# 54rt1n/shardmerge

Hardware: AMD Instinct MI355X
Metric: merged-weight GB/s per GPU + % HBM roofline, Llama-3-70B 3-way FFT merge (higher is better)
Workload: dtype f32; 1 GPU; Llama-3-70B block tensors, this rank's 1/8 slice (9 per block x 10 blocks), K=3 finetunes, bf16 in/out, resident in HBM; workload_id=llama3-70b-slice, k=3, parallelism=tensor-partition x1 (no data-path collective), streams_per_gpu=8

## Files before the change

shardmerge_amd/csrc/sm_capi.inc:

```

struct smhip_ctx {
    smhip::Pipeline<SM_BACKEND> pipe;
    explicit smhip_ctx(int device) : pipe(device) {}
};

#define SM_GUARD(ctx)                      \
    if (!(ctx)) return SMHIP_ERR_ARG;      \
    (ctx)->pipe.err.clear();
#define SM_FINISH(ctx, rc)                                                        \
    do {                                                                          \
        int rc__ = (rc);                                                          \
        if (rc__ == SMHIP_OK && !(ctx)->pipe.be.ok()) {                           \
            (ctx)->pipe.err = (ctx)->pipe.be.error();                             \
            rc__ = SMHIP_ERR_HIP;                                                 \
        }                                                                         \
        return rc__;                                                              \
    } while (0)

template <class Desc, class Scalars>
static int delta_tensor_check(smhip_ctx* ctx, const char* op, const Desc* d, const void* out, const float* delta_out,
                              bool need_base, Scalars scalars) {
    auto bad = [&](const char* what) { return ctx->pipe.fail(SMHIP_ERR_ARG, std::string(op) + ": " + what); };
    if (!d) return bad("null descriptor");
    if (d->k < 1 || d->k > SMHIP_MAX_MODELS) return bad("k out of range (1..16)");
// ... 350 lines not shown
                             void* stream) {
    SM_GUARD(ctx);
    if (!x || !norm_out) return ctx->pipe.fail(SMHIP_ERR_ARG, "bad argument");
    if (dtype < SMHIP_BF16 || dtype > SMHIP_F32) return ctx->pipe.fail(SMHIP_ERR_ARG, "bad dtype");
    ctx->pipe.stream = stream;
    const int rc0 = ctx->pipe.reserve(1, 1);
    if (rc0) SM_FINISH(ctx, rc0);
    smhip::SigDesc sg{x, base, dtype, 1.f};
    double out = 0;
    if (!ctx->pipe.run_serial_norms(&sg, 1, n, &out))
        return ctx->pipe.fail(SMHIP_ERR_ARG, "reference_cpu norm: inputs must be 16-byte aligned");
    *norm_out = (float)out;
    SM_FINISH(ctx, SMHIP_OK);
}

int smhip_debug_option(smhip_ctx* ctx, const char* key, long value) {
    SM_GUARD(ctx);
    if (key && std::string(key) == "aten_overlap") { ctx->pipe.aten_overlap = value != 0; return SMHIP_OK; }
    if (key && std::string(key) == "emf_max_sample") { ctx->pipe.emf_max_sample = value >= 1 && value <= 4096 ? (int)value : smhip::EMF_MAX_SAMPLE; return SMHIP_OK; }
    if (key && std::string(key) == "aten_serial") { ctx->pipe.aten_serial = value != 0; return SMHIP_OK; }
    if (key && std::string(key) == "class_norms") { ctx->pipe.class_norms_mode = value >= 0 && value <= 2 ? (int)value : 1; return SMHIP_OK; }
    if (key && std::string(key) == "cand_cap") { ctx->pipe.debug_cand_cap = value > 0 ? (uint32_t)value : 0u; return SMHIP_OK; }
    if (key && std::string(key) == "sel_chunks") { ctx->pipe.debug_sel_chunks = value > 0 ? (uint32_t)value : 0u; return SMHIP_OK; }
    if (key && std::string(key) == "sel_flush_always") { ctx->pipe.debug_flush_always = value != 0; return SMHIP_OK; }
    if (key && std::string(key) == "fuse_norms") { ctx->pipe.fuse_norms = value != 0; return SMHIP_OK; }
    if (key && std::string(key) == "noise_seed") { ctx->pipe.noise_seed_base = (uint32_t)value; return SMHIP_OK; }
    if (key && std::string(key) == "spectral_intermediates") { ctx->pipe.spectral_inter = value != 0; return SMHIP_OK; }
    if (key && std::string(key) == "fuse_spec_norm") { ctx->pipe.fuse_spec_norm = value != 0; return SMHIP_OK; }
    if (key && std::string(key) == "sel_wgs_per_cu") { ctx->pipe.sel_wgs_per_cu = value > 0 ? (int)value : 5; return SMHIP_OK; }
    if (key && std::string(key) == "pair1d") { ctx->pipe.pair1d_enabled = value != 0; return SMHIP_OK; }
    if (key && std::string(key) == "spec_cull") { ctx->pipe.spec_cull = value != 0; return SMHIP_OK; }
    if (key && std::string(key) == "spec_min_bins") { ctx->pipe.spec_min_bins = value >= 0 ? (size_t)value : (size_t)1 << 20; return SMHIP_OK; }
    if (key && std::string(key) == "dftp_pairs") { ctx->pipe.dftp_pairs_enabled = value != 0; return SMHIP_OK; }
    if (key && std::string(key) == "f2s_pair") { ctx->pipe.f2s_pair = value != 0; return SMHIP_OK; }
    if (key && std::string(key) == "f1_multi") { ctx->pipe.f1_multi = value != 0; return SMHIP_OK; }
    if (key && std::string(key) == "force_bluestein") { ctx->pipe.debug_force_bluestein = value != 0; return SMHIP_OK; }
    if (key && std::string(key) == "force_split") { ctx->pipe.debug_force_split = value > 1 && value <= smhip::DFTP_MAX_P ? (int)value : 0; return SMHIP_OK; }
    if (key && std::string(key) == "fold_columns") { ctx->pipe.fold_enabled = value != 0; return SMHIP_OK; }
    if (key && std::string(key) == "della_slab_rows") { ctx->pipe.della_slab_rows = value > 0 ? (size_t)value : 0; return SMHIP_OK; }
    if (key && std::string(key) == "fold_min_rows") { ctx->pipe.fold_min_rows = value > 0 ? (int)value : SM_FOLD_MIN_ROWS; return SMHIP_OK; }
    return ctx->pipe.fail(SMHIP_ERR_ARG, "unknown debug option");
}

int smhip_debug_query(smhip_ctx* ctx, const char* key, long* value) {
    SM_GUARD(ctx);
    if (!key || !value) return SMHIP_ERR_ARG;
    if (std::string(key) == "spec_hit") { *value = ctx->pipe.last_spec_verdict(); SM_FINISH(ctx, SMHIP_OK); }
    if (std::string(key) == "spec_checked" || std::string(key) == "spec_hits") {
        unsigned long long c = 0, h = 0;
        ctx->pipe.spec_totals(&c, &h);
        *value = (long)(std::string(key) == "spec_hits" ? h : c);
        SM_FINISH(ctx, SMHIP_OK);
    }
    if (std::string(key) == "aten_fast" || std::string(key) == "aten_group" || std::string(key) == "aten_slow") {
        unsigned long long v3[3];
        ctx->pipe.aten_stats(1, v3);
        *value = (long)v3[std::string(key) == "aten_fast" ? 0 : std::string(key) == "aten_group" ? 1 : 2];
        SM_FINISH(ctx, SMHIP_OK);
    }
    return ctx->pipe.fail(SMHIP_ERR_ARG, "unknown debug query");
}

int smhip_profile_enable(smhip_ctx* ctx, int on) { SM_GUARD(ctx); ctx->pipe.be.profile_enable(on != 0); return SMHIP_OK; }
int smhip_profile_reset(smhip_ctx* ctx) { SM_GUARD(ctx); ctx->pipe.be.profile_reset(); return SMHIP_OK; }
int smhip_profile_count(smhip_ctx* ctx) { return ctx ? ctx->pipe.be.profile_count() : 0; }
int smhip_profile_get(smhip_ctx* ctx, int i, const char** name, uint64_t* launches, double* total_ms) {
    SM_GUARD(ctx);
    return ctx->pipe.be.profile_get(i, name, launches, total_ms) ? SMHIP_OK : SMHIP_ERR_ARG;
}

}
```

shardmerge_amd/csrc/sm_kernels.hpp:

```cpp
#pragma once
#include <cmath>
#include <cstring>

#include "fft_engine.hpp"
#include "sm_aten_core.hpp"

namespace smhip {

struct cf4 { float x, y, z, w; };
struct u32x4 { uint32_t x, y, z, w; };

enum { DT_BF16 = 0, DT_F16 = 1, DT_F32 = 2 };

struct SigDesc {
    const void* x;
    const void* base;
    int dtype;
    float prescale;
};

SM_HD uint32_t umax(uint32_t a, uint32_t b) { return a > b ? a : b; }
SM_HD float u2f(uint32_t u) { float f; memcpy(&f, &u, 4); return f; }
SM_HD uint32_t f2u(float f) { uint32_t u; memcpy(&u, &f, 4); return u; }
SM_HD float bf16_to_f(uint32_t h) { return u2f(h << 16); }
// ... 882 lines not shown
    }
}

#ifndef SM_COL_THREADS
#define SM_COL_THREADS 512
#endif
constexpr int f2_bins_for(int T, int N = 1 << 30) {
    if (T == 64 && N <= 256) return 8;
    return (SM_COL_THREADS / (2 * T)) > 1 ? (SM_COL_THREADS / (2 * T) > 8 ? 8 : SM_COL_THREADS / (2 * T)) : 1;
}
#ifndef SM_I1_THREADS
constexpr int i1_bins_for(int T) { return 2; }
#else
constexpr int i1_bins_for(int T) { return (SM_I1_THREADS / T) > 2 ? ((SM_I1_THREADS / T) > 16 ? 16 : (SM_I1_THREADS / T)) : 2; }
#endif
template <class P> constexpr int f2_bins() { if constexpr (P::is_static) return f2_bins_for(P::T, P::N); else return 1; }
template <class P> constexpr int i1_bins() { if constexpr (P::is_static) return i1_bins_for(P::T); else return 2; }

struct F2SParams {
    FftPlanDev plan;
    const cf4* t1;
    int pitch4;
    int R, C, Cb;
    int role_a;
    float scale;
    float* re; float* im;
    unsigned long long* hist;
    int slab, Cb_real, Rfull;
    size_t slab_elems;
    double* im_partials;
    SliceGrid sl;
    int two;
    const cf4* t1_2; int role_a_2; float scale_2; float* re_2;
};
template <class P> constexpr int f2s_groups() {
    if constexpr (P::is_static) return f2_nsig_for(P::T) == 2 ? 2 * f2_bins_for(P::T, P::N) : 1; else return 1;
}

#ifndef SM_F2S_ILV
#define SM_F2S_ILV 1
#endif
constexpr int F2S_ILV = SM_F2S_ILV;
#ifndef SM_F2S_DIRECT
#define SM_F2S_DIRECT 0
#endif
template <class P, int G> constexpr int f2s_direct() {
    if constexpr (!P::is_static) return 0;
    else {
        constexpr int R0 = P::radix(0);
        constexpr bool ok = F2S_ILV == 1 && (G == 1 || G == 2) && P::npass >= 2 && P::T % 2 == 0 && R0 % 2 == 0 &&
                            (P::N / R0) % 2 == 0 && (EMAX / R0) * R0 * P::T >= P::N;
        return ok ? (SM_F2S_DIRECT & 3) : 0;
    }
}
template <class P, int G, bool FOLD = false, class Ex>
SM_HD void k_f2s(Ex& ex, const F2SParams& p) {
    if constexpr (FOLD && !fold_col_plan<P>()) { return; } else {
    typename Ex::template State<FftState> st;
    ex.init(st);
    float* lds = ex.lds() + LDS_SCRATCH_FLOATS;
    const FftPlanDev& pl = p.plan;
    const int T = plan_T<P>(pl), R = plan_N<P>(pl);
    const int LF = plan_lds<P>(pl);
    constexpr int XG = G >= 8 ? 1 : 8 / G;
    int bid_in_slice;
    const int slice = slice_of(ex, p.sl, bid_in_slice);
    int sig2 = 0;
    const int lbid = p.two ? pick_signal(2, bid_in_slice, XG, sig2) : xcd_remap(bid_in_slice, XG);
    const cf4* const t1 = (sig2 ? p.t1_2 : p.t1) + slice * p.sl.t1_stride;
    const size_t pl_off = slice * p.sl.plane_stride;
    const int role_a_ = sig2 ? p.role_a_2 : p.role_a;
    const float scale_ = sig2 ? p.scale_2 : p.scale;
    float* const re_ = sig2 ? p.re_2 : p.re;
    const int kbase = lbid * G;
    if (kbase >= p.Cb) {
        if (p.im_partials) ex.each(st, [&](int tid, FftState&) { if (tid == 0) p.im_partials[ex.bid()] = 0.0; });
        return;
    }
    const int nthreads = G * T;
    const int half = R / 2;
    uint32_t* lhist = (uint32_t*)(lds + G * LF);

    constexpr int DIRECT = f2s_direct<P, G>();
    if constexpr ((DIRECT & 1) != 0) {
        constexpr int R0 = P::radix(0), MB0 = EMAX / R0, nb0 = P::N / R0;
        ex.each(st, [&](int tid, FftState& s) {
            const int g = tid / T, t = tid % T;
            const int k2 = kbase + g;
            const int kc = k2 < p.Cb ? k2 : p.Cb - 1;
            const int par = t & 1;
            static_for<0, MB0>([&](auto m_c) {
                constexpr int m = decltype(m_c)::value;
                const bool live = (t + m * T) < nb0 && k2 < p.Cb;
                static_for<0, R0 / 2>([&](auto q_c) {
                    constexpr int q = decltype(q_c)::value;
                    const int pm = live ? (t >> 1) + m * (T / 2) + q * nb0 + par * (nb0 / 2) : 0;
                    cf4 v;
#if defined(SM_DIAG_NOMEM)
                    v = cf4{(float)q, (float)t, 1.f, (float)kc};
#else
                    if constexpr (FOLD) v = t1[(size_t)(kc / p.slab) * p.slab_elems + (size_t)pm * p.slab + (kc % p.slab)];
                    else v = t1[(size_t)pm * p.pitch4 + kc];
#endif
                    s.xr[m * R0 + 2 * q] = live ? v.x : 0.f; s.xi[m * R0 + 2 * q] = live ? v.y : 0.f;
                    s.xr[m * R0 + 2 * q + 1] = live ? v.z : 0.f; s.xi[m * R0 + 2 * q + 1] = live ? v.w : 0.f;
                });
// ... 55 lines not shown
#pragma unroll
                for (int c = 0; c < 4; ++c) {
                    const int k1 = 4 * (t + u * T) + c;
                    if (k1 < R) o[4 * u + c] = l[lpad(k1)];
                }
            }
        });

    ex.each(st, [&](int tid, FftState& s) {
        const int g = tid / T, t = tid % T;
        const int k2 = kbase + g;
        s.red[0] = 0.0;
        if (k2 >= p.Cb) return;
        const float sc = scale_;
        size_t poff = (size_t)k2 * R;
        int kreal = k2;
        if constexpr (FOLD) { kreal = fold_bin(k2, p.slab, p.Cb_real, R, p.Rfull, poff); if (kreal < 0) return; }
        const uint32_t w = (uint32_t)bin_weight(kreal, p.C);
        float* dre = re_ + pl_off + poff;
        float* dim = p.im + pl_off + poff;
        float imsq = 0.f;
        if constexpr ((DIRECT & 2) != 0) {
            constexpr int RL = P::radix(P::npass - 1), MBL = EMAX / RL, NsL = P::N / RL;
            static_for<0, MBL>([&](auto m_c) {
                constexpr int m = decltype(m_c)::value;
                const int j = t + m * T;
                if (j < NsL) {
                    static_for<0, RL>([&](auto i_c) {
                        constexpr int i = decltype(i_c)::value, e = m * RL + i;
                        const float vr = s.xr[e] * sc;
#if defined(SM_DIAG_NOMEM)
                        if (vr == 12345.678f)
#endif
                        dre[j + i * NsL] = vr;
                        if (role_a_) {
                            const float vi = s.xi[e] * sc;
#if defined(SM_DIAG_NOMEM)
                            if (vi == 12345.678f)
#endif
                            dim[j + i * NsL] = vi;
                            imsq += vi * vi;
                        }
                        if (p.hist) ex.lds_atomic_add(&lhist[(f2u(vr) & 0x7fffffffu) >> 20], w);
                    });
                }
            });
        } else
#pragma unroll
        for (int u = 0; u < EMAX / 4; ++u) {
            const int k0 = 4 * (t + u * T);
            if (k0 + 3 < R && (R & 3) == 0) {
                cf4 vr = {s.xr[4 * u] * sc, s.xr[4 * u + 1] * sc, s.xr[4 * u + 2] * sc, s.xr[4 * u + 3] * sc};
#if defined(SM_DIAG_NOMEM)
                if (vr.x == 12345.678f)
#endif
                *(cf4*)(dre + k0) = vr;
                if (role_a_) {
                    cf4 vi = {s.xi[4 * u] * sc, s.xi[4 * u + 1] * sc, s.xi[4 * u + 2] * sc, s.xi[4 * u + 3] * sc};
#if defined(SM_DIAG_NOMEM)
                    if (vi.x == 12345.678f)
#endif
                    *(cf4*)(dim + k0) = vi;
                    imsq += vi.x * vi.x + vi.y * vi.y + vi.z * vi.z + vi.w * vi.w;
                }
            } else {
#pragma unroll
                for (int c = 0; c < 4; ++c) {
                    if (k0 + c < R) {
                        dre[k0 + c] = s.xr[4 * u + c] * sc;
                        if (role_a_) { const float vi = s.xi[4 * u + c] * sc; dim[k0 + c] = vi; imsq += vi * vi; }
                    }
                }
            }
            if (p.hist) {
#pragma unroll
                for (int c = 0; c < 4; ++c) {
                    if (k0 + c < R) {
                        const uint32_t key = f2u(s.xr[4 * u + c] * sc) & 0x7fffffffu;
                        ex.lds_atomic_add(&lhist[key >> 20], w);
                    }
                }
            }
        }
        s.red[0] = (double)imsq * (double)w;
    });
    if (p.hist) {
        ex.sync();
        ex.each(st, [&](int tid, FftState&) {
            for (int h = tid; h < HIST1_BINS; h += nthreads) {
                const uint32_t v = lhist[h];
                if (v) ex.global_atomic_add(&p.hist[h], (unsigned long long)v);
            }
        });
    }
    if (p.im_partials) {
        ex.sync();
        ex.template block_sum<1>(st, [&](const double* tot) { p.im_partials[ex.bid()] = tot[0]; });
    }
    }
}

template <class Ex>
SM_HD void k_f2_r1(Ex& ex, const F2Params& p) {
// ... 1435 lines not shown
            sr += qr; si += qi2;
        }
        s.red[0] = sr; s.red[1] = si;
    });
    ex.template block_sum<2>(st, [&](const double* tot) {
        p.partials[2 * (size_t)ex.bid()] = tot[0];
        p.partials[2 * (size_t)ex.bid() + 1] = tot[1];
    });
}

SM_HD uint32_t hash_u32(uint32_t x) {
    x ^= x >> 16; x *= 0x7feb352du; x ^= x >> 15; x *= 0x846ca68bu; x ^= x >> 16;
    return x;
}
SM_HD float model_noise(uint32_t seed, size_t i, float sigma) {
    const uint32_t h1 = hash_u32((uint32_t)i * 2u + 1u + seed * 0x9e3779b9u) ^ hash_u32((uint32_t)(i >> 31) + seed);
    const uint32_t h2 = hash_u32(h1 + 0x68bc21ebu);
    if ((h2 >> 24) < 21u) return 0.f;
    const float s4 = (float)(h1 & 0xffffu) + (float)(h1 >> 16) + (float)(h2 & 0xffffu) + (float)(hash_u32(h2) >> 16);
    return sigma * 1.7320508f * (s4 * (1.0f / 65536.0f) - 2.0f);
}

struct SpecRescaleParams {
    const float* re; const float* im;
    float* dre; float* dim;
    int R, C, Cb;
    int vec4;
    float thr;
    float scale;
    float sigma; uint32_t seed;
    unsigned long long* hist;
    int chunks;
    double* im_partials;
};
template <class Ex>
SM_HD void k_spec_rescale(Ex& ex, const SpecRescaleParams& p) {
    typename Ex::template State<EmptyState> st;
    ex.init(st);
    uint32_t* lh = (uint32_t*)(ex.lds() + LDS_SCRATCH_FLOATS);
    const int nt = ex.nthreads();
    const size_t total = (size_t)p.Cb * p.R;
    const size_t nquad = (total + 3) / 4;
    const WeightRanges wr = weight_ranges(p.R, p.C, p.Cb);
    if (p.hist) {
        ex.each(st, [&](int tid, EmptyState&) { for (int b = tid; b < HIST1_BINS; b += nt) lh[b] = 0; });
        ex.sync();
    }
    ex.each(st, [&](int tid, EmptyState& s) {
        double imacc = 0.0;
        const size_t start = (size_t)ex.bid() * p.chunks * nt;
        for (int c = 0; c < p.chunks; ++c) {
            const size_t qi = start + (size_t)c * nt + tid;
            if (qi >= nquad) break;
            const size_t i0 = 4 * qi;
            float a[4], b[4] = {0.f, 0.f, 0.f, 0.f};
            const int n = load_quad(p.re, i0, total, p.vec4, a);
            if (p.im) load_quad(p.im, i0, total, p.vec4, b);
            float r[4], im[4];
#pragma unroll
            for (int e = 0; e < 4; ++e) {
                r[e] = (fabsf(a[e]) < p.thr) ? model_noise(p.seed, i0 + e, p.sigma) : a[e] * p.scale;
                im[e] = b[e] * p.scale;
            }
            if (p.vec4) {
                cf4 v = {r[0], r[1], r[2], r[3]};
                *(cf4*)(p.dre + i0) = v;
                if (p.im) { cf4 vi = {im[0], im[1], im[2], im[3]}; *(cf4*)(p.dim + i0) = vi; }
            } else {
                for (int e = 0; e < n; ++e) { p.dre[i0 + e] = r[e]; if (p.im) p.dim[i0 + e] = im[e]; }
            }
            if (p.hist) {
#pragma unroll
                for (int e = 0; e < 4; ++e)
                    if (e < n) ex.lds_atomic_add(&lh[(f2u(r[e]) & 0x7fffffffu) >> 20], weight_at(wr, i0 + e));
            }
            if (p.im_partials) {
                float q = 0.f;
#pragma unroll
                for (int e = 0; e < 4; ++e)
                    if (e < n) q += (float)weight_at(wr, i0 + e) * im[e] * im[e];
                imacc += q;
            }
        }
        s.red[0] = imacc;
    });
    if (p.hist) {
        ex.sync();
        ex.each(st, [&](int tid, EmptyState&) {
            for (int b = tid; b < HIST1_BINS; b += nt) {
                const uint32_t v = lh[b];
                if (v) ex.global_atomic_add(&p.hist[b], (unsigned long long)v);
            }
        });
    }
    if (p.im_partials) {
        ex.sync();
        ex.template block_sum<1>(st, [&](const double* tot) { p.im_partials[ex.bid()] = tot[0]; });
    }
}

constexpr int NORMS_MAX = 16;
constexpr int NORMS_K = 8;
// ... 1210 lines not shown
```

shardmerge_amd/csrc/sm_pipeline.hpp:

```cpp
#pragma once
#include <algorithm>
#include <cmath>
#include <cstdio>
#include <map>
#include <string>
#include <vector>

#include "../../include/shardmerge_hip.h"
#include "sm_kernels.hpp"
#include "sm_aten_norm.hpp"
#include "sm_bluestein.hpp"
#include "sm_lora.hpp"
#include "sm_ties.hpp"
#include "sm_dare.hpp"
#include "sm_breadcrumbs.hpp"
#include "sm_geo.hpp"
#include "sm_sce.hpp"
#include "sm_della.hpp"
#include "sm_consensus.hpp"

namespace smhip {

#define SM_KERNEL_TAG(Tag, ParamsT, NAME, CALL)                                      \
    struct Tag {                                                                     \
// ... 292 lines not shown
};

struct ProfEntry { std::string name; uint64_t launches = 0; double ms = 0; };

inline size_t round_up(size_t v, size_t m) { return (v + m - 1) / m * m; }

struct PairOut {
    void* out = nullptr; int out_mode = OUT_F32;
    const void* base = nullptr; int base_dtype = DT_BF16;
    float post = 1.f;
    int ifft_policy = 1;
};

template <class B>
class Pipeline {
  public:
    B be;
    std::string err;
    void* stream = nullptr;
    uint32_t debug_cand_cap = 0;
    uint32_t debug_sel_chunks = 0;
    bool debug_flush_always = false;
    bool spec_cull = true;
    size_t spec_min_bins = 1 << 20;
    bool dftp_pairs_enabled = true;
    int debug_force_split = 0;
    int sel_wgs_per_cu = 5;
    bool safe_select = false;
    uint32_t noise_seed_base = 0;
    bool spectral_inter = true;
    bool f2s_pair = true;
    size_t f2s_pair_max_bins = (size_t)64 << 20;
    bool f1_multi = true;
    bool fuse_spec_norm = true;
    float noise_sigma = 1.2e-7f;

    explicit Pipeline(int device) : be(device) {}
    ~Pipeline() {
        for (auto& kv : plans_) if (kv.second.dev.tw) be.free((void*)kv.second.dev.tw);
        for (Buffer* b : {&cand_, &t1_, &small_, &tmpA_, &tmpB_, &tmpC_, &fullS_, &saveR_, &saveI_, &aten_, &emf_, &lora_, &dora_, &ties_}) if (b->p) be.free(b->p);
        for (Buffer& b : pool_) if (b.p) be.free(b.p);
        if (mail_) be.free_host(mail_);
        for (Buffer& b : inter_) if (b.p) be.free(b.p);
        for (Buffer& b : rowspec_) if (b.p) be.free(b.p);
        for (Buffer& b : tr_) if (b.p) be.free(b.p);
        for (auto& kv : rough_tw_) if (kv.second) be.free(kv.second);
        for (auto& kv : blue_) { if (kv.second.chirp) be.free(kv.second.chirp); if (kv.second.filt) be.free(kv.second.filt); }
    }

    int fail(int code, const std::string& msg) { err = msg; return code; }

    int get_plan(int N, FftPlanDev& out) {
        auto it = plans_.find(N);
        if (it == plans_.end()) {
            HostPlan hp;
            int T;
            std::vector<int> rad;
            if (plan_shape(N, T, rad)) {
                hp.ok = true;
                hp.dev.N = N; hp.dev.T = T; hp.dev.npass = (int)rad.size();
                for (int i = 0; i < MAX_PASSES; ++i) hp.dev.radix[i] = i < (int)rad.size() ? rad[i] : 1;
                hp.dev.cx = plan_uses_cx(N) ? 1 : 0;
                hp.dev.lds_floats = hp.dev.cx ? (int)round_up((size_t)2 * (N + (N >> 4) + 1), 32)
                                              : (int)round_up((size_t)lpad(N) + 1, 32);
                std::vector<cf2> tw(N);
                for (int j = 0; j < N; ++j) {
// ... 383 lines not shown
            return SMHIP_OK;
        }
        const int xgs = p.ilv > p.nb ? p.ilv / p.nb : 1;
        const bool joint = joint_rows(g);
        const int nlaunch = joint ? 1 : g.batch;
        if (joint) p.R = g.R * g.rough / 2;
        const int grid = (int)round_up((size_t)(p.R + p.nb - 1) / p.nb, 8 * xgs);
        if (multi && (nlaunch != 1 || g.rough > 1 || (size_t)grid * 2 * nm > PART_DOUBLES || !p.vec)) return SMHIP_ERR_ARG;
        if ((size_t)grid * 2 * nlaunch > PART_DOUBLES) return fail(SMHIP_ERR_SHAPE, "too many rows");
        const size_t lds = (LDS_SCRATCH_FLOATS + (size_t)p.nb * p.plan.lds_floats) * 4;
        cf4* const t1base = p.t1;
        double* const pbase = p.partials;
        if (multi) {
            for (int i = 0; i < nm; ++i) multi->partials[i] = pbase + (size_t)i * 2 * grid;
            multi->b_off = (long long)((size_t)g.C * dt_size(sig.dtype));
            p.sigs = *multi;
            launch_fft<KF1>(p.plan, grid * nm, p.nb * p.plan.T, lds, p, true);
            if (grid_out) *grid_out = grid;
            return SMHIP_OK;
        }
        for (int bi = 0; bi < nlaunch; ++bi) {
            p.a = sig_at(a, (size_t)bi * g.R * g.C); p.b = sig_at(b, (size_t)bi * g.R * g.C);
            p.t1 = t1base + (size_t)bi * (g.t1_slice / 2);
            p.partials = pbase + (size_t)bi * 2 * grid;
            if (blue) { F1BParams q; q.f = p; q.bt = bt; launch_fft<KF1B>(p.plan, grid, p.plan.T, lds, q); }
            else launch_fft<KF1>(p.plan, grid, p.nb * p.plan.T, lds, p, p.vec != 0);
        }
        if (grid_out) *grid_out = grid * nlaunch;
        if (g.rough > 1) return run_dftp(g, t1base, true, F2S_ILV, g.pitch4, g.t1_slice / 2, false);
        return SMHIP_OK;
    }
    struct F2SSecond { const void* t1; bool role_a; float scale; };
    int run_f2s(const Geo& g, bool role_a, float scale, bool hist, const void* t1buf = nullptr, int* im_parts = nullptr,
                const F2SSecond* second = nullptr) {
        F2SParams p;
        p.two = 0; p.t1_2 = nullptr; p.role_a_2 = 0; p.scale_2 = 0.f; p.re_2 = nullptr;
        if (second) {
            if (g.batch != 1 || second->role_a == role_a) return fail(SMHIP_ERR_ARG, "internal: paired column pass");
            p.two = 1; p.t1_2 = (const cf4*)second->t1; p.role_a_2 = second->role_a ? 1 : 0; p.scale_2 = second->scale;
            p.re_2 = plane(g, second->role_a ? P_REA : P_REB);
        }
        const int nsg = second ? 2 : 1;
        const int Rt = g.R / g.fold;
        int rc = get_plan(Rt, p.plan);
        if (rc) return rc;
        p.t1 = (const cf4*)(t1buf ? t1buf : t1_.p); p.pitch4 = g.pitch4 * g.fold; p.R = Rt; p.C = g.C;
        p.Cb = g.fold == 4 ? 4 * g.pitch4 : g.C / 2 + 1;
        p.slab = g.pitch4; p.Cb_real = g.C / 2 + 1; p.Rfull = g.R; p.slab_elems = fold_slab_elems(g, true);
        p.role_a = role_a ? 1 : 0; p.scale = scale;
        p.re = plane(g, role_a ? P_REA : P_REB); p.im = plane(g, P_IMA);
        p.hist = hist ? d_hist() : nullptr;
        const bool st = is_static_plan(p.plan);
        const int G = st ? (f2_nsig_for(p.plan.T) == 2 ? 2 * f2_bins_for(p.plan.T, p.plan.N) : 1) : 1;
        const int xg = G >= 8 ? 1 : 8 / G;
        const int grid = (int)round_up((size_t)(p.Cb + G - 1) / G, 8 * xg) * nsg;
        const size_t lds = (LDS_SCRATCH_FLOATS + (size_t)G * p.plan.lds_floats + HIST1_BINS) * 4;
        const bool any_a = role_a || (second && second->role_a);
        const bool want_im = im_parts && any_a && (size_t)grid * g.batch <= PART_IM_DOUBLES;
        if (im_parts) *im_parts = want_im ? grid * g.batch : -1;
        p.im_partials = want_im ? d_part_im() : nullptr;
        if (g.fold == 4) { launch_fft<KF2SQ>(p.plan, grid, G * p.plan.T, lds, p); return SMHIP_OK; }
        if (g.batch > 1) { p.sl.wgs = grid; p.sl.t1_stride = g.t1_slice / 2; p.sl.plane_stride = (size_t)(g.C / 2 + 1) * g.R; }
        launch_fft<KF2S>(p.plan, grid * g.batch, G * p.plan.T, lds, p);
        return SMHIP_OK;
    }
    void run_spec_norm(const Geo& g, const float* re, const float* im, const float* thr, double& sre, double& sim) {
        const size_t total = (size_t)g.Cb * g.R;
        SpecNormParams q;
        q.re = re; q.im = im; q.R = g.R; q.C = g.Cw; q.Cb = g.Cb; q.vec4 = vec4(g); q.thr = thr;
        q.chunks = pick_chunks((total + 3) / 4, 256, 8, 8);
        int grid = stream_grid((total + 3) / 4, 256, q.chunks);
        while ((size_t)grid * 2 > PART_DOUBLES) { q.chunks *= 2; grid = stream_grid((total + 3) / 4, 256, q.chunks); }
        q.partials = d_part();
        be.template launch<KSpecNorm>(grid, 256, LDS_SCRATCH_FLOATS * 4, q, stream);
        SumPartialsParams sp;
        sp.partials = d_part(); sp.nparts = grid; sp.out = mail_->norm2;
        be.template launch<KSumPartials>(1, 1024, LDS_SCRATCH_FLOATS * 4, sp, stream);
        PublishParams pp;
        pp.flags = d_flags(); pp.thr = d_thr(0); pp.consts = d_consts(); pp.mail = mail_; pp.zero_flags = nullptr;
        be.template launch<KPublish>(1, 64, LDS_SCRATCH_FLOATS * 4, pp, stream);
        be.sync(stream);
        sre = mail_->norm2[0]; sim = mail_->norm2[1];
    }
    void run_spec_rescale(const Geo& g, const float* re, const float* im, float thr, float scale, bool role_a, bool hist,
                          int* im_parts = nullptr) {
        const size_t total = (size_t)g.Cb * g.R;
        SpecRescaleParams q;
        q.re = re; q.im = role_a ? im : nullptr;
        q.dre = plane(g, role_a ? P_REA : P_REB); q.dim = plane(g, P_IMA);
        q.R = g.R; q.C = g.Cw; q.Cb = g.Cb; q.vec4 = vec4(g);
        q.thr = thr; q.scale = scale; q.sigma = noise_sigma; q.seed = ++noise_seed_;
        q.hist = hist ? d_hist() : nullptr;
        q.chunks = pick_chunks((total + 3) / 4, 256, 8, 8);
        const int grid = stream_grid((total + 3) / 4, 256, q.chunks);
        const bool want_im = im_parts && role_a && (size_t)grid <= PART_IM_DOUBLES;
        if (im_parts) *im_parts = want_im ? grid : -1;
        q.im_partials = want_im ? d_part_im() : nullptr;
        be.template launch<KSpecRescale>(grid, 256, (LDS_SCRATCH_FLOATS + HIST1_BINS) * 4, q, stream);
    }
    void run_spec_norm_fused(int sel_parts, int im_parts, double& sre, double& sim) {
        SumsqCandParams sc;
        sc.cand = cand_lists(); sc.thr = d_thr(1); sc.partials = d_part() + 4 * (size_t)sel_parts;
        be.template launch<KSumsqCand>(CAND_GRID, 256, LDS_SCRATCH_FLOATS * 4, sc, stream);
        SumSpecParams sp;
        sp.part4 = d_part(); sp.n4 = sel_parts + CAND_GRID; sp.part1 = d_part_im(); sp.n1 = im_parts; sp.out = mail_->norm2;
        sp.zero_u32 = d_candctr(); sp.zero_u32_count = 3;
        be.template launch<KSumSpec>(1, 1024, LDS_SCRATCH_FLOATS * 4, sp, stream);
        PublishParams pp;
        pp.flags = d_flags(); pp.thr = d_thr(0); pp.consts = d_consts(); pp.mail = mail_; pp.zero_flags = nullptr;
        be.template launch<KPublish>(1, 64, LDS_SCRATCH_FLOATS * 4, pp, stream);
        be.sync(stream);
        sre = mail_->norm2[0]; sim = mail_->norm2[1];
    }

    void read_norms(int grid, double& na, double& nb) {
        SumPartialsParams sp;
        sp.partials = d_part(); sp.nparts = grid; sp.out = mail_->norm2;
        be.template launch<KSumPartials>(1, 1024, LDS_SCRATCH_FLOATS * 4, sp, stream);
        be.sync(stream);
        na = std::sqrt(mail_->norm2[0]); nb = std::sqrt(mail_->norm2[1]);
    }

    int run_f2(const Geo& g, float scale0, float scale1, int swap, bool hist) {
        F2Params p;
        int rc = get_plan(g.R, p.plan);
        if (rc) return rc;
        if (g.R == 1) {
            p.slab = g.pitch4; p.Cb_real = g.C / 2 + 1; p.Rfull = 1; p.slab_elems = 0;
            p.t1 = (const cf4*)t1_.p; p.pitch4 = g.pitch4; p.ilv = 1; p.R = 1; p.C = g.C; p.Cb = g.C / 2 + 1; p.nsig = 2;
            p.swap = swap; p.scale[0] = scale0; p.scale[1] = scale1;
// ... 496 lines not shown
        std::vector<char> used(m, 0);
        std::vector<float> corr((size_t)m * m, 0.f);
        for (int i = 0; i < m; ++i)
            for (int j = i + 1; j < m; ++j) corr[(size_t)i * m + j] = norms[i] * norms[j];
        for (;;) {
            float best = INFINITY;
            bool any = false;
            for (int i = 0; i < m; ++i)
                for (int j = i + 1; j < m; ++j)
                    if (!used[i] && !used[j]) { any = true; best = std::min(best, std::fabs(corr[(size_t)i * m + j])); }
            if (!any) break;
            int bx = -1, by = -1;
            for (int i = 0; i < m && bx < 0; ++i)
                for (int j = i + 1; j < m; ++j)
                    if (!used[i] && !used[j] && std::fabs(corr[(size_t)i * m + j]) == best) { bx = i; by = j; break; }
            if (bx < 0) break;
            out.emplace_back(bx, by);
            used[bx] = used[by] = 1;
        }
        for (int i = 0; i < m; ++i)
            if (!used[i]) out.emplace_back(i, -1);
    }

    struct Slot {
        SigDesc sig;
        double weight;
        double norm;
        bool spectral = false;
        int re_id = -1, im_id = -1;
        float thr = 0.f;
        double spec_scale = 1.0;
        double post = 1.0;
        int rows_id = -1;
    };
    int materialise(const Geo& g, Slot& s, std::vector<char>& inter_busy) {
        if (!s.spectral) return SMHIP_OK;
        const size_t n = (size_t)g.R * g.C;
        int id = -1;
        for (size_t q = 0; q < inter_.size(); ++q) if (!inter_busy[q]) { id = (int)q; break; }
        if (id < 0) { inter_.emplace_back(); inter_busy.push_back(0); id = (int)inter_.size() - 1; }
        int rc = ensure(inter_[id], n * sizeof(float));
        if (rc) return rc;
        inter_busy[id] = 1;
        PairOut po;
        po.out = inter_[id].p; po.out_mode = OUT_F32; po.post = (float)s.post;
        if ((rc = run_inverse(g, (const float*)pool_[s.re_id].p, (const float*)pool_[s.im_id].p, nullptr, po, nullptr, s.thr))) return rc;
        pool_release(s.re_id); pool_release(s.im_id);
        s.spectral = false; s.re_id = s.im_id = -1;
        s.sig = SigDesc{inter_[id].p, nullptr, DT_F32, 1.f};
        return SMHIP_OK;
    }

    bool run_delta_norms(const smhip_layer_desc& d, size_t n, std::vector<Slot>& stack) {
        if (d.k > NORMS_K || d.in_dtype == DT_F32 || (n % 8) != 0) return false;
        DeltaNormsParams p;
        p.k = d.k; p.dtype = d.in_dtype; p.n = n;
        p.ubase[0] = p.ubase[1] = nullptr;
        int nb = 0;
        for (int i = 0; i < NORMS_K; ++i) { p.ft[i] = d.finetune[i < d.k ? i : 0]; p.base_of[i] = 0; }
        for (int i = 0; i < d.k; ++i) {
            if (!d.base[i] || !aligned16(d.base[i]) || !aligned16(d.finetune[i])) return false;
            int j = 0;
            while (j < nb && p.ubase[j] != d.base[i]) ++j;
            if (j == nb) { if (nb == 2) return false; p.ubase[nb++] = d.base[i]; }
            p.base_of[i] = j;
        }
        p.chunks = pick_chunks(n / 8, 256, 4, 8);
        int grid = stream_grid(n / 8, 256, p.chunks);
        while ((size_t)grid * NORMS_MAX > PART_DOUBLES) { p.chunks *= 2; grid = stream_grid(n / 8, 256, p.chunks); }
        p.partials = d_part();
        be.template launch<KDeltaNorms>(grid, 256, LDS_SCRATCH_FLOATS * 4, p, stream);
        SumNParams sp;
        sp.partials = d_part(); sp.nparts = grid; sp.out = mail_->norm2;
        be.template launch<KSumPartialsN>(1, 256, LDS_SCRATCH_FLOATS * 4, sp, stream);
        be.sync(stream);
// ... 410 lines not shown
                return fail(SMHIP_ERR_NONFINITE, buf);
            }
        }
        {
            float acc = 0.f;
            for (int i = 0; i < d.k; ++i) acc += norms32[i];
            mean = (double)(acc / (float)d.k);
        }
        const double target_norm = mean + d.target_norm_offset;
        rp.target_norm = target_norm;
        double cull_pct = d.cull_start_pct;

        std::vector<char> inter_busy(inter_.size(), 0);
        for (size_t q = 0; q < pool_.size(); ++q) {
            bool working = false;
            for (int i = 0; i < 4; ++i) working = working || pidx_[i] == (int)q;
            pool_busy_[q] = working ? 1 : 0;
        }
        noise_seed_ = noise_seed_base;
        int step = 0;
        int round_idx = 0;
        int pair_idx = 0;
        int deferred_step = -1;
        bool deferred_cut = false, deferred_cull = false;
        while (stack.size() > 1) {
            const int m = (int)stack.size();
            std::vector<std::pair<int, int>> pairs;
            correlated_pairs_least(norms32, m, pairs);
            std::vector<Slot> next;
            const bool last_round = (pairs.size() == 1 && pairs[0].second >= 0);
            bool any_pair = false;
            for (auto& pr : pairs) any_pair = any_pair || pr.second >= 0;
            if (!any_pair) { check_flags(false, false); return fail(SMHIP_ERR_NONFINITE, "no pair can be formed (non-finite norms)"); }
            for (auto& pr : pairs) {
                const int x = pr.first, y = pr.second;
                if (step < SMHIP_MAX_PAIRS) { rp.step_x[step] = x; rp.step_y[step] = y; }
                if (y < 0) {
                    next.push_back(stack[x]);
                    if (step < SMHIP_MAX_PAIRS) rp.step_branch[step] = SMHIP_BRANCH_CARRY;
                    ++step;
                    continue;
                }
                Slot A = stack[x], Bs = stack[y];
                const double a_w = stack[x].weight, b_w = stack[y].weight;
                if (A.norm < 0 || Bs.norm < 0) return fail(SMHIP_ERR_ARG, "internal: norm unknown");
                double na = (double)(float)A.norm, nb = (double)(float)Bs.norm;
                bool swapped = false;
                if (std::fabs(na) < std::fabs(nb)) { std::swap(A, Bs); std::swap(na, nb); swapped = true; }
                const double ca = std::fabs(na / target_norm), cb = std::fabs(nb / target_norm);
                const double ratio = cb / (ca + 1e-10);
                PairOut po;
                float* inter = nullptr;
                const bool linear = (nb / (na + 1e-10)) < d.b;
                const bool slerp_proper = !(ca < 1e-6) && !(cb < 1e-6 || ratio < 0.1) && !(nb < 1e-4 || na < 1e-4) && !linear;
                if (last_round) {
                    po = fin;
                } else if (slerp_proper && spectral_ok) {
                } else {
                    int id = -1;
                    for (size_t q = 0; q < inter_.size(); ++q) if (!inter_busy[q]) { id = (int)q; break; }
                    if (id < 0) { inter_.emplace_back(); inter_busy.push_back(0); id = (int)inter_.size() - 1; }
                    Buffer* bb = &inter_[id];
                    if ((rc = ensure(*bb, n * sizeof(float)))) return rc;
                    inter_busy[id] = 1;
                    inter = (float*)bb->p;
                    po.out = inter; po.out_mode = OUT_F32; po.post = 1.f;
// ... 25 lines not shown
                    pa.ifft_policy = 0;
                    if ((rc = pair_arith(A.sig, Bs.sig, R, C, (float)s, (float)(w * s), 1.0, 1, pa, na, nb, &g))) return rc;
                    if (dtmp) {
                        SigDesc ds{dtmp, nullptr, DT_F32, 1.f}, none{nullptr, nullptr, DT_F32, 1.f};
                        run_combine(ds, none, 1.f, 0.f, n, nullptr, &fin, false);
                    }
                    f1_ready = false;
                } else {
                    branch = SMHIP_BRANCH_SLERP;
                    const double t = a_w / (a_w + b_w);
                    if (nb < 1e-4 || na < 1e-4) {
                        SigDesc none{nullptr, nullptr, DT_F32, 1.f};
                        const float sc = (float)(target_norm / na);
                        if (last_round) run_combine(A.sig, none, sc, 0.f, n, delta_out, &po, false);
                        else run_combine(A.sig, none, sc, 0.f, n, inter, nullptr, false);
                        branch = SMHIP_BRANCH_EARLY_V0;
                    } else if (linear) {
                        branch = SMHIP_BRANCH_LINEAR;
                        int grid;
                        if ((rc = run_f1(g, A.sig, Bs.sig, grid))) return rc;
                        f1_ready = false;
                        if ((rc = run_f2_linear(g, (float)(1.0 / na), (float)(1.0 / nb), (float)t))) return rc;
                        PairOut ps = po;
                        ps.post = (float)target_norm;
                        float* dtmp = nullptr;
                        if (last_round && delta_out) { ps = PairOut(); ps.out = delta_out; ps.post = (float)target_norm; dtmp = delta_out; }
                        if ((rc = run_inverse(g, plane(g, P_RER), plane(g, P_IMA), nullptr, ps, last_round ? nullptr : &inv_grid))) return rc;
                        if (dtmp) {
                            SigDesc ds{dtmp, nullptr, DT_F32, 1.f}, none{nullptr, nullptr, DT_F32, 1.f};
                            run_combine(ds, none, 1.f, 0.f, n, nullptr, &fin, false);
                        }
                    } else {
                        int im_parts = -1;
                        const bool any_spec = stack[x].spectral || stack[y].spectral ||
                                              (stack[x].rows_id >= 0 && stack[y].rows_id >= 0);
                        const bool fused1d = !any_spec && pair1d_ok(g);
                        if (fused1d) {
                            f1_ready = false;
                        } else if (!any_spec) {
                            if (!(f1_ready && d.k == 2)) {
                                int grid;
                                if ((rc = run_f1(g, stack[x].sig, stack[y].sig, grid))) return rc;
                            }
                            f1_ready = false;
                            const float s0 = (float)(1.0 / (double)(float)stack[x].norm);
                            const float s1 = (float)(1.0 / (double)(float)stack[y].norm);
                            if ((rc = run_f2(g, s0, s1, swapped ? 1 : 0, d.cutoff_pct > 0))) return rc;
                        } else {
                            f1_ready = false;
                            int* imp = (!last_round && spectral_ok && fuse_spec_norm) ? &im_parts : nullptr;
                            if (f2s_pair && g.batch == 1 && g.fold == 1 && (size_t)g.Cb * g.R <= f2s_pair_max_bins &&
                                !stack[x].spectral && !stack[y].spectral &&
                                stack[x].rows_id >= 0 && stack[y].rows_id >= 0) {
                                const bool xa = !swapped;
                                F2SSecond sec{rowspec_[stack[y].rows_id].p, !xa, (float)(1.0 / (double)(float)stack[y].norm)};
                                if ((rc = run_f2s(g, xa, (float)(1.0 / (double)(float)stack[x].norm), d.cutoff_pct > 0,
                                                  rowspec_[stack[x].rows_id].p, imp, &sec))) return rc;
                            } else
                            for (int side = 0; side < 2; ++side) {
                                const Slot& in = side == 0 ? stack[x] : stack[y];
                                const bool role_a = (side == 0) != swapped;
                                int* ip = role_a ? imp : nullptr;
                                if (in.spectral) {
                                    run_spec_rescale(g, (const float*)pool_[in.re_id].p, (const float*)pool_[in.im_id].p, in.thr,
                                                     (float)in.spec_scale, role_a, d.cutoff_pct > 0, ip);
                                } else if (in.rows_id >= 0) {
                                    if ((rc = run_f2s(g, role_a, (float)(1.0 / (double)(float)in.norm), d.cutoff_pct > 0,
                                                      rowspec_[in.rows_id].p, ip))) return rc;
                                } else {
                                    if ((rc = run_f1_rowpairs(g, in.sig))) return rc;
                                    if ((rc = run_f2s(g, role_a, (float)(1.0 / (double)(float)in.norm), d.cutoff_pct > 0, nullptr, ip))) return rc;
                                }
                            }
                        }
                        bool have_cull;
                        int sel_parts = 0;
                        const bool fused_norm = im_parts > 0 && !safe_select && cull_pct > 0;
                        if (fused1d) have_cull = cull_pct > 0;
                        else spectral_blend(g, BLEND_SLERP, t, d.t_sum, d.cutoff_pct, cull_pct, 1, true, have_cull,
                                            fused_norm ? &sel_parts : nullptr, std::min(pair_idx++, 6));
                        for (int side = 0; side < 2; ++side) {
                            Slot& in = side == 0 ? stack[x] : stack[y];
                            if (in.spectral) { pool_release(in.re_id); pool_release(in.im_id); in.re_id = in.im_id = -1; }
                        }
                        if (!last_round && spectral_ok) {
                            double sre, sim;
                            if (fused_norm && sel_parts > 0) run_spec_norm_fused(sel_parts, im_parts, sre, sim);
                            else run_spec_norm(g, plane(g, P_RER), plane(g, P_IMA), have_cull ? d_thr(1) : nullptr, sre, sim);
                            read_blend_info(&info, d.cutoff_pct > 0, have_cull, true, true);
                            const double ssum = (sre + sim) / ((double)R * (double)C);
                            out_spectral = true;
                            spec_slot = Slot();
                            spec_slot.spectral = true;
                            spec_slot.re_id = pidx_[P_RER]; spec_slot.im_id = pidx_[P_IMA];
                            spec_slot.thr = have_cull ? mail_->thr[1] : 0.f;
                            const double nrm_exact = target_norm * std::sqrt(ssum);
                            const double bias = ref_norms ? aten_gauss_norm_ratio((double)n, nrm_exact / std::sqrt((double)n)) : 1.0;
                            spec_slot.spec_scale = ssum > 0 ? 1.0 / (std::sqrt(ssum) * bias) : 1.0;
                            spec_slot.post = target_norm;
                            spec_slot.norm = nrm_exact * bias;
                            spec_slot.sig = SigDesc{nullptr, nullptr, DT_F32, 1.f};
                            const int r1 = pool_acquire(g.plane_floats * sizeof(float));
                            const int r2 = pool_acquire(g.plane_floats * sizeof(float));
                            if (r1 < 0 || r2 < 0) return SMHIP_ERR_NOMEM;
                            pidx_[P_RER] = r1; pidx_[P_IMA] = r2;
                        } else {
                        PairOut ps = po;
                        ps.post = (float)target_norm;
                        float* dtmp = nullptr;
                        if (last_round && delta_out) { ps = PairOut(); ps.out = delta_out; ps.post = (float)target_norm; dtmp = delta_out; }
                        if (fused1d) {
                            if ((rc = run_pair1d(g, A.sig, Bs.sig, na, nb, t, d.t_sum, d.cutoff_pct, cull_pct, ps,
                                                 last_round ? nullptr : &inv_grid))) return rc;
                        } else
                        if ((rc = run_inverse(g, plane(g, P_RER), plane(g, P_IMA), have_cull ? d_thr(1) : nullptr, ps,
                                              last_round ? nullptr : &inv_grid))) return rc;
                        if (dtmp) {
                            SigDesc ds{dtmp, nullptr, DT_F32, 1.f}, none{nullptr, nullptr, DT_F32, 1.f};
                            run_combine(ds, none, 1.f, 0.f, n, nullptr, &fin, false);
                        }
                        if (last_round) {
                            deferred_step = step; deferred_cut = d.cutoff_pct > 0; deferred_cull = have_cull;
                        } else {
                            read_blend_info(&info, d.cutoff_pct > 0, have_cull, true);
                        }
                        }
                    }
                }
                if (branch == SMHIP_BRANCH_SLERP || branch == SMHIP_BRANCH_LINEAR) { info.t = a_w / (a_w + b_w); info.cull_pct = cull_pct; }
                if (step < SMHIP_MAX_PAIRS) { rp.step_branch[step] = branch; rp.step_info[step] = info; }
                ++step;
                for (size_t q = 0; q < inter_.size(); ++q)
                    if (inter_[q].p && (inter_[q].p == stack[x].sig.x || inter_[q].p == stack[y].sig.x)) inter_busy[q] = 0;
                if (!last_round && out_spectral) {
                    spec_slot.weight = (a_w + b_w) / 2.0;
                    next.push_back(spec_slot);
// ... 807 lines not shown
```

Baseline: 87.17 GB/s.

## Defer storing the role-A imaginary spectrum plane and recompute it lazily

The role-A column FFT pass can now skip writing the imaginary plane when the fused spectral-norm path is used and the next round's opponent is likely to take role A. If the Im plane is needed later (rescale as role A, materialise, or the unfused norm path), it is recomputed from the retained row spectrum with an Im-only column pass. This saves one full-plane f32 write per pair plus a pool buffer, at the cost of a possible recompute FFT pass when the prediction is wrong.

New measurement: 87.88 GB/s (median of 6 runs). Within noise of the previous version (+0.8%).

```diff
diff --git a/shardmerge_amd/csrc/sm_capi.inc b/shardmerge_amd/csrc/sm_capi.inc
--- a/shardmerge_amd/csrc/sm_capi.inc
+++ b/shardmerge_amd/csrc/sm_capi.inc
@@ -406,6 +406,7 @@
     if (key && std::string(key) == "spec_cull") { ctx->pipe.spec_cull = value != 0; return SMHIP_OK; }
     if (key && std::string(key) == "spec_min_bins") { ctx->pipe.spec_min_bins = value >= 0 ? (size_t)value : (size_t)1 << 20; return SMHIP_OK; }
     if (key && std::string(key) == "dftp_pairs") { ctx->pipe.dftp_pairs_enabled = value != 0; return SMHIP_OK; }
+    if (key && std::string(key) == "lazy_im") { ctx->pipe.lazy_im = value >= 0 && value <= 2 ? (int)value : 1; return SMHIP_OK; }
     if (key && std::string(key) == "f2s_pair") { ctx->pipe.f2s_pair = value != 0; return SMHIP_OK; }
     if (key && std::string(key) == "f1_multi") { ctx->pipe.f1_multi = value != 0; return SMHIP_OK; }
     if (key && std::string(key) == "force_bluestein") { ctx->pipe.debug_force_bluestein = value != 0; return SMHIP_OK; }
@@ -426,6 +427,8 @@
         *value = (long)(std::string(key) == "spec_hits" ? h : c);
         SM_FINISH(ctx, SMHIP_OK);
     }
+    if (std::string(key) == "im_deferred") { *value = (long)ctx->pipe.im_deferred_; SM_FINISH(ctx, SMHIP_OK); }
+    if (std::string(key) == "im_recovered") { *value = (long)ctx->pipe.im_recovered_; SM_FINISH(ctx, SMHIP_OK); }
     if (std::string(key) == "aten_fast" || std::string(key) == "aten_group" || std::string(key) == "aten_slow") {
         unsigned long long v3[3];
         ctx->pipe.aten_stats(1, v3);
diff --git a/shardmerge_amd/csrc/sm_kernels.hpp b/shardmerge_amd/csrc/sm_kernels.hpp
--- a/shardmerge_amd/csrc/sm_kernels.hpp
+++ b/shardmerge_amd/csrc/sm_kernels.hpp
@@ -938,6 +938,7 @@
     SliceGrid sl;
     int two;
     const cf4* t1_2; int role_a_2; float scale_2; float* re_2;
+    int store_im, store_re;
 };
 template <class P> constexpr int f2s_groups() {
     if constexpr (P::is_static) return f2_nsig_for(P::T) == 2 ? 2 * f2_bins_for(P::T, P::N) : 1; else return 1;
@@ -978,6 +979,7 @@
     const int role_a_ = sig2 ? p.role_a_2 : p.role_a;
     const float scale_ = sig2 ? p.scale_2 : p.scale;
     float* const re_ = sig2 ? p.re_2 : p.re;
+    const bool store_im_ = p.store_im != 0, store_re_ = p.store_re != 0;
     const int kbase = lbid * G;
     if (kbase >= p.Cb) {
         if (p.im_partials) ex.each(st, [&](int tid, FftState&) { if (tid == 0) p.im_partials[ex.bid()] = 0.0; });
@@ -1099,13 +1101,13 @@
 #if defined(SM_DIAG_NOMEM)
                         if (vr == 12345.678f)
 #endif
-                        dre[j + i * NsL] = vr;
+                        if (store_re_) dre[j + i * NsL] = vr;
                         if (role_a_) {
                             const float vi = s.xi[e] * sc;
 #if defined(SM_DIAG_NOMEM)
                             if (vi == 12345.678f)
 #endif
-                            dim[j + i * NsL] = vi;
+                            if (store_im_) dim[j + i * NsL] = vi;
                             imsq += vi * vi;
                         }
                         if (p.hist) ex.lds_atomic_add(&lhist[(f2u(vr) & 0x7fffffffu) >> 20], w);
@@ -1121,21 +1123,21 @@
 #if defined(SM_DIAG_NOMEM)
                 if (vr.x == 12345.678f)
 #endif
-                *(cf4*)(dre + k0) = vr;
+                if (store_re_) *(cf4*)(dre + k0) = vr;
                 if (role_a_) {
                     cf4 vi = {s.xi[4 * u] * sc, s.xi[4 * u + 1] * sc, s.xi[4 * u + 2] * sc, s.xi[4 * u + 3] * sc};
 #if defined(SM_DIAG_NOMEM)
                     if (vi.x == 12345.678f)
 #endif
-                    *(cf4*)(dim + k0) = vi;
+                    if (store_im_) *(cf4*)(dim + k0) = vi;
                     imsq += vi.x * vi.x + vi.y * vi.y + vi.z * vi.z + vi.w * vi.w;
                 }
             } else {
 #pragma unroll
                 for (int c = 0; c < 4; ++c) {
                     if (k0 + c < R) {
-                        dre[k0 + c] = s.xr[4 * u + c] * sc;
-                        if (role_a_) { const float vi = s.xi[4 * u + c] * sc; dim[k0 + c] = vi; imsq += vi * vi; }
+                        if (store_re_) dre[k0 + c] = s.xr[4 * u + c] * sc;
+                        if (role_a_) { const float vi = s.xi[4 * u + c] * sc; if (store_im_) dim[k0 + c] = vi; imsq += vi * vi; }
                     }
                 }
             }
@@ -2637,6 +2639,7 @@
     unsigned long long* hist;
     int chunks;
     double* im_partials;
+    int store_im;
 };
 template <class Ex>
 SM_HD void k_spec_rescale(Ex& ex, const SpecRescaleParams& p) {
@@ -2670,9 +2673,9 @@
             if (p.vec4) {
                 cf4 v = {r[0], r[1], r[2], r[3]};
                 *(cf4*)(p.dre + i0) = v;
-                if (p.im) { cf4 vi = {im[0], im[1], im[2], im[3]}; *(cf4*)(p.dim + i0) = vi; }
+                if (p.im && p.store_im) { cf4 vi = {im[0], im[1], im[2], im[3]}; *(cf4*)(p.dim + i0) = vi; }
             } else {
-                for (int e = 0; e < n; ++e) { p.dre[i0 + e] = r[e]; if (p.im) p.dim[i0 + e] = im[e]; }
+                for (int e = 0; e < n; ++e) { p.dre[i0 + e] = r[e]; if (p.im && p.store_im) p.dim[i0 + e] = im[e]; }
             }
             if (p.hist) {
 #pragma unroll
diff --git a/shardmerge_amd/csrc/sm_pipeline.hpp b/shardmerge_amd/csrc/sm_pipeline.hpp
--- a/shardmerge_amd/csrc/sm_pipeline.hpp
+++ b/shardmerge_amd/csrc/sm_pipeline.hpp
@@ -348,6 +348,8 @@
     bool f2s_pair = true;
     size_t f2s_pair_max_bins = (size_t)64 << 20;
     bool f1_multi = true;
+    int lazy_im = 1;
+    unsigned long long im_deferred_ = 0, im_recovered_ = 0;
     bool fuse_spec_norm = true;
     float noise_sigma = 1.2e-7f;
 
@@ -797,8 +799,9 @@
     }
     struct F2SSecond { const void* t1; bool role_a; float scale; };
     int run_f2s(const Geo& g, bool role_a, float scale, bool hist, const void* t1buf = nullptr, int* im_parts = nullptr,
-                const F2SSecond* second = nullptr) {
+                const F2SSecond* second = nullptr, bool* defer_im = nullptr, float* im_only = nullptr) {
         F2SParams p;
+        if (im_only && (!role_a || second || hist || im_parts || defer_im)) return fail(SMHIP_ERR_ARG, "internal: Im-only column pass");
         p.two = 0; p.t1_2 = nullptr; p.role_a_2 = 0; p.scale_2 = 0.f; p.re_2 = nullptr;
         if (second) {
             if (g.batch != 1 || second->role_a == role_a) return fail(SMHIP_ERR_ARG, "internal: paired column pass");
@@ -813,7 +816,8 @@
         p.Cb = g.fold == 4 ? 4 * g.pitch4 : g.C / 2 + 1;
         p.slab = g.pitch4; p.Cb_real = g.C / 2 + 1; p.Rfull = g.R; p.slab_elems = fold_slab_elems(g, true);
         p.role_a = role_a ? 1 : 0; p.scale = scale;
-        p.re = plane(g, role_a ? P_REA : P_REB); p.im = plane(g, P_IMA);
+        p.re = plane(g, role_a ? P_REA : P_REB); p.im = im_only ? im_only : plane(g, P_IMA);
+        p.store_re = im_only ? 0 : 1; p.store_im = 1;
         p.hist = hist ? d_hist() : nullptr;
         const bool st = is_static_plan(p.plan);
         const int G = st ? (f2_nsig_for(p.plan.T) == 2 ? 2 * f2_bins_for(p.plan.T, p.plan.N) : 1) : 1;
@@ -824,6 +828,7 @@
         const bool want_im = im_parts && any_a && (size_t)grid * g.batch <= PART_IM_DOUBLES;
         if (im_parts) *im_parts = want_im ? grid * g.batch : -1;
         p.im_partials = want_im ? d_part_im() : nullptr;
+        if (defer_im) { *defer_im = *defer_im && want_im; p.store_im = *defer_im ? 0 : 1; }
         if (g.fold == 4) { launch_fft<KF2SQ>(p.plan, grid, G * p.plan.T, lds, p); return SMHIP_OK; }
         if (g.batch > 1) { p.sl.wgs = grid; p.sl.t1_stride = g.t1_slice / 2; p.sl.plane_stride = (size_t)(g.C / 2 + 1) * g.R; }
         launch_fft<KF2S>(p.plan, grid * g.batch, G * p.plan.T, lds, p);
@@ -861,6 +866,7 @@
         const bool want_im = im_parts && role_a && (size_t)grid <= PART_IM_DOUBLES;
         if (im_parts) *im_parts = want_im ? grid : -1;
         q.im_partials = want_im ? d_part_im() : nullptr;
+        q.store_im = 1;
         be.template launch<KSpecRescale>(grid, 256, (LDS_SCRATCH_FLOATS + HIST1_BINS) * 4, q, stream);
     }
     void run_spec_norm_fused(int sel_parts, int im_parts, double& sre, double& sim) {
@@ -1423,7 +1429,23 @@
         double spec_scale = 1.0;
         double post = 1.0;
         int rows_id = -1;
+        int im_rows_id = -1;
+        float im_scale = 0.f;
     };
+    int recover_im(const Geo& g, int rows_id, float scale, float* dst) {
+        if (rows_id < 0 || rows_id >= (int)rowspec_.size() || !rowspec_[rows_id].p) return fail(SMHIP_ERR_ARG, "internal: no row spectrum to take an Im plane from");
+        ++im_recovered_;
+        return run_f2s(g, true, scale, false, rowspec_[rows_id].p, nullptr, nullptr, nullptr, dst);
+    }
+    int ensure_im(const Geo& g, Slot& s) {
+        if (!s.spectral || s.im_id >= 0) return SMHIP_OK;
+        const int id = pool_acquire(g.plane_floats * sizeof(float));
+        if (id < 0) return SMHIP_ERR_NOMEM;
+        const int rc = recover_im(g, s.im_rows_id, s.im_scale, (float*)pool_[id].p);
+        if (rc) { pool_release(id); return rc; }
+        s.im_id = id; s.im_rows_id = -1;
+        return SMHIP_OK;
+    }
     int materialise(const Geo& g, Slot& s, std::vector<char>& inter_busy) {
         if (!s.spectral) return SMHIP_OK;
         const size_t n = (size_t)g.R * g.C;
@@ -1432,6 +1454,7 @@
         if (id < 0) { inter_.emplace_back(); inter_busy.push_back(0); id = (int)inter_.size() - 1; }
         int rc = ensure(inter_[id], n * sizeof(float));
         if (rc) return rc;
+        if ((rc = ensure_im(g, s))) return rc;
         inter_busy[id] = 1;
         PairOut po;
         po.out = inter_[id].p; po.out_mode = OUT_F32; po.post = (float)s.post;
@@ -1908,6 +1931,18 @@
             bool any_pair = false;
             for (auto& pr : pairs) any_pair = any_pair || pr.second >= 0;
             if (!any_pair) { check_flags(false, false); return fail(SMHIP_ERR_NONFINITE, "no pair can be formed (non-finite norms)"); }
+            std::vector<std::pair<int, int>> next_pairs;
+            if (!last_round) correlated_pairs_least(norms32, (int)pairs.size(), next_pairs);
+            auto opponent_takes_role_a = [&](int pos) {
+                for (auto& q : next_pairs) {
+                    if (q.second < 0 || (q.first != pos && q.second != pos)) continue;
+                    const int o = q.first == pos ? q.second : q.first;
+                    if (pairs[o].second >= 0) return false;
+                    const Slot& s = stack[pairs[o].first];
+                    return !s.spectral && s.rows_id >= 0 && (double)(float)s.norm >= target_norm;
+                }
+                return false;
+            };
             for (auto& pr : pairs) {
                 const int x = pr.first, y = pr.second;
                 if (step < SMHIP_MAX_PAIRS) { rp.step_x[step] = x; rp.step_y[step] = y; }
@@ -1999,6 +2034,9 @@
                         }
                     } else {
                         int im_parts = -1;
+                        bool defer_im = false;
+                        int defer_rows = -1;
+                        float defer_scale = 0.f;
                         const bool any_spec = stack[x].spectral || stack[y].spectral ||
                                               (stack[x].rows_id >= 0 && stack[y].rows_id >= 0);
                         const bool fused1d = !any_spec && pair1d_ok(g);
@@ -2016,24 +2054,29 @@
                         } else {
                             f1_ready = false;
                             int* imp = (!last_round && spectral_ok && fuse_spec_norm) ? &im_parts : nullptr;
+                            const Slot& ra = swapped ? stack[y] : stack[x];
+                            defer_rows = ra.rows_id; defer_scale = (float)(1.0 / (double)(float)ra.norm);
+                            defer_im = lazy_im != 0 && imp && !safe_select && cull_pct > 0 && !ra.spectral && ra.rows_id >= 0 &&
+                                       (lazy_im == 2 || opponent_takes_role_a((int)next.size()));
                             if (f2s_pair && g.batch == 1 && g.fold == 1 && (size_t)g.Cb * g.R <= f2s_pair_max_bins &&
                                 !stack[x].spectral && !stack[y].spectral &&
                                 stack[x].rows_id >= 0 && stack[y].rows_id >= 0) {
                                 const bool xa = !swapped;
                                 F2SSecond sec{rowspec_[stack[y].rows_id].p, !xa, (float)(1.0 / (double)(float)stack[y].norm)};
                                 if ((rc = run_f2s(g, xa, (float)(1.0 / (double)(float)stack[x].norm), d.cutoff_pct > 0,
-                                                  rowspec_[stack[x].rows_id].p, imp, &sec))) return rc;
+                                                  rowspec_[stack[x].rows_id].p, imp, &sec, &defer_im))) return rc;
                             } else
                             for (int side = 0; side < 2; ++side) {
-                                const Slot& in = side == 0 ? stack[x] : stack[y];
+                                Slot& in = side == 0 ? stack[x] : stack[y];
                                 const bool role_a = (side == 0) != swapped;
                                 int* ip = role_a ? imp : nullptr;
                                 if (in.spectral) {
+                                    if (role_a && (rc = ensure_im(g, in))) return rc;
                                     run_spec_rescale(g, (const float*)pool_[in.re_id].p, (const float*)pool_[in.im_id].p, in.thr,
                                                      (float)in.spec_scale, role_a, d.cutoff_pct > 0, ip);
                                 } else if (in.rows_id >= 0) {
                                     if ((rc = run_f2s(g, role_a, (float)(1.0 / (double)(float)in.norm), d.cutoff_pct > 0,
-                                                      rowspec_[in.rows_id].p, ip))) return rc;
+                                                      rowspec_[in.rows_id].p, ip, nullptr, role_a ? &defer_im : nullptr))) return rc;
                                 } else {
                                     if ((rc = run_f1_rowpairs(g, in.sig))) return rc;
                                     if ((rc = run_f2s(g, role_a, (float)(1.0 / (double)(float)in.norm), d.cutoff_pct > 0, nullptr, ip))) return rc;
@@ -2053,13 +2096,21 @@
                         if (!last_round && spectral_ok) {
                             double sre, sim;
                             if (fused_norm && sel_parts > 0) run_spec_norm_fused(sel_parts, im_parts, sre, sim);
-                            else run_spec_norm(g, plane(g, P_RER), plane(g, P_IMA), have_cull ? d_thr(1) : nullptr, sre, sim);
+                            else {
+                                if (defer_im) {
+                                    if ((rc = recover_im(g, defer_rows, defer_scale, plane(g, P_IMA)))) return rc;
+                                    defer_im = false; ++im_deferred_;
+                                }
+                                run_spec_norm(g, plane(g, P_RER), plane(g, P_IMA), have_cull ? d_thr(1) : nullptr, sre, sim);
+                            }
                             read_blend_info(&info, d.cutoff_pct > 0, have_cull, true, true);
                             const double ssum = (sre + sim) / ((double)R * (double)C);
                             out_spectral = true;
                             spec_slot = Slot();
                             spec_slot.spectral = true;
-                            spec_slot.re_id = pidx_[P_RER]; spec_slot.im_id = pidx_[P_IMA];
+                            spec_slot.re_id = pidx_[P_RER];
+                            if (defer_im) { spec_slot.im_rows_id = defer_rows; spec_slot.im_scale = defer_scale; ++im_deferred_; }
+                            else spec_slot.im_id = pidx_[P_IMA];
                             spec_slot.thr = have_cull ? mail_->thr[1] : 0.f;
                             const double nrm_exact = target_norm * std::sqrt(ssum);
                             const double bias = ref_norms ? aten_gauss_norm_ratio((double)n, nrm_exact / std::sqrt((double)n)) : 1.0;
@@ -2068,7 +2119,7 @@
                             spec_slot.norm = nrm_exact * bias;
                             spec_slot.sig = SigDesc{nullptr, nullptr, DT_F32, 1.f};
                             const int r1 = pool_acquire(g.plane_floats * sizeof(float));
-                            const int r2 = pool_acquire(g.plane_floats * sizeof(float));
+                            const int r2 = defer_im ? pidx_[P_IMA] : pool_acquire(g.plane_floats * sizeof(float));
                             if (r1 < 0 || r2 < 0) return SMHIP_ERR_NOMEM;
                             pidx_[P_RER] = r1; pidx_[P_IMA] = r2;
                         } else {
```
